# yamoling/lle

Hardware: AMD Instinct MI355X
Metric: env-steps/s (agents x envs x steps/s), level-6 batch 65536 (higher is better)
Workload: dtype u8

## Files before the change

### lle_amd/csrc/kernel_common.hpp

```cpp
#pragma once
#include <hip/hip_runtime.h>
#include <stdint.h>
#include <stdlib.h>

#include "kernels.h"
#include "obs_stream.hpp"
#include "step_logic.hpp"
#include "tables.h"

namespace lle {

enum Mode : int { MODE_STEP = 0, MODE_RESET = 1, MODE_SET_STATE = 2, MODE_OBSERVE = 3, MODE_SOURCES = 4, MODE_ENV_SOURCES = 5 };

__device__ __forceinline__ uint64_t wave_sum_u64(uint64_t v) {
#pragma unroll
    for (int o = 32; o >= 1; o >>= 1) {
        uint32_t lo = __shfl_xor((uint32_t)v, o, 64);
        uint32_t hi = __shfl_xor((uint32_t)(v >> 32), o, 64);
        v += ((uint64_t)hi << 32) | lo;
    }
    return v;
}

struct StepCounts { uint32_t steps, gems, exits, died, invalid, resets, bonus; };
__device__ __forceinline__ uint32_t wave_sum_u32(uint32_t v) {
#pragma unroll
    for (int o = 32; o >= 1; o >>= 1) v += __shfl_xor(v, o, 64);
    return v;
}
__device__ __forceinline__ int64_t stats_preload(const int64_t* __restrict__ stats, uint32_t wave_id, uint32_t lane) {
    return lane < 8 ? stats[(int64_t)wave_id * 8 + lane] : 0;
}
__device__ __forceinline__ void flush_stats(int64_t* __restrict__ stats, uint32_t wave_id, const StepCounts& c, int A, uint32_t lane,
                                            bool preloaded = false, int64_t old = 0) {
    const int64_t steps = wave_sum_u32(c.steps), gems = wave_sum_u32(c.gems), exits = wave_sum_u32(c.exits);
    const int64_t died = wave_sum_u32(c.died), invalid = wave_sum_u32(c.invalid), resets = wave_sum_u32(c.resets);
    const int64_t bonus = wave_sum_u32(c.bonus);
    const int64_t v = lane == 0 ? steps : lane == 1 ? steps * A : lane == 2 ? gems : lane == 3 ? exits : lane == 4 ? died
                    : lane == 5 ? invalid : lane == 6 ? resets : gems + exits - died + bonus;
    if (preloaded) {
        if (lane < 8) stats[(int64_t)wave_id * 8 + lane] = old + v;
    } else if (lane == 0) {
        int64_t* out = stats + (int64_t)wave_id * 8;
        out[0] += steps; out[1] += steps * A; out[2] += gems; out[3] += exits; out[4] += died;
        out[5] += invalid; out[6] += resets; out[7] += gems + exits - died + bonus;
    }
}

template <int AM>
__device__ __forceinline__ void store_u16_record(uint16_t* __restrict__ base, int64_t env, const uint32_t (&v)[AM]) {
    uint32_t* __restrict__ w = reinterpret_cast<uint32_t*>(base) + env * (AM / 2);
#pragma unroll
    for (int k = 0; k < AM / 2; k++) w[k] = (v[2 * k] & 0xFFFFu) | (v[2 * k + 1] << 16);
}
template <int AM>
__device__ __forceinline__ void load_u8_record(const uint8_t* __restrict__ base, int64_t env, uint32_t (&out)[AM]) {
    const uint32_t* __restrict__ w = reinterpret_cast<const uint32_t*>(base) + env * (AM / 4);
#pragma unroll
    for (int k = 0; k < AM / 4; k++) {
        const uint32_t v = w[k];
#pragma unroll
        for (int q = 0; q < 4; q++) out[4 * k + q] = (v >> (8 * q)) & 0xFFu;
    }
}
template <int AM>
__device__ __forceinline__ void store_u8_record(uint8_t* __restrict__ base, int64_t env, const uint32_t (&v)[AM]) {
    uint32_t* __restrict__ w = reinterpret_cast<uint32_t*>(base) + env * (AM / 4);
#pragma unroll
    for (int k = 0; k < AM / 4; k++)
        w[k] = (v[4 * k] & 0xFFu) | ((v[4 * k + 1] & 0xFFu) << 8) | ((v[4 * k + 2] & 0xFFu) << 16) | (v[4 * k + 3] << 24);
}

}
```

### lle_amd/csrc/step_kernel.hpp

```cpp
#pragma once
#include "kernel_common.hpp"
#include "partial_stream.hpp"
#include "step_lanes.hpp"

namespace lle {


__device__ __forceinline__ EnvOutputs load_uniform(const EnvOutputs* p) {
    static_assert(sizeof(EnvOutputs) == 64, "one s_load_dwordx16");
    typedef uint32_t u32x16 __attribute__((ext_vector_type(16)));
    u32x16 w;
    asm volatile("s_load_dwordx16 %0, %1, 0x0\n\ts_waitcnt lgkmcnt(0)" : "=s"(w) : "s"(p) : "memory");
    EnvOutputs o;
    __builtin_memcpy(&o, &w, sizeof o);
    return o;
}

constexpr size_t KERNARG_ENV_OUT = ((sizeof(BatchPtrs) + alignof(LaunchArgs) - 1) / alignof(LaunchArgs)) * alignof(LaunchArgs) + offsetof(LaunchArgs, out);
__device__ __forceinline__ const EnvOutputs* kernarg_env_out() {
    return reinterpret_cast<const EnvOutputs*>((const char*)__builtin_amdgcn_kernarg_segment_ptr() + KERNARG_ENV_OUT);
}

__device__ __forceinline__ uint32_t park_uniform(uint32_t s) {
    uint32_t v;
// ... 167 lines not shown
    const uint32_t head2_lo = (HEAD && PES) ? hdr->pes_head2_lo : 0u, head2_n = (HEAD && PES && head_n) ? head2_n_map : 0u;
    uint4 head_v = {0u, 0u, 0u, 0u};
    if (HEAD) {
        const uint32_t q_lay = hdr->off_cell_lay, q_lds = hdr->lds_table_bytes, q_ig = initp->gems;
        const uint64_t q_ib = initp->bits;
        asm("" : "+s"(head_lo) : "s"(h_HW), "s"(h_obs_stride), "s"(h_n_chunks), "s"(h_D), "s"(h_enabled), "s"(h_off_cell_meta), "s"(h_off_dyn), "s"(h_off_template),
                                 "s"(head_n_map), "s"(q_lay), "s"(q_lds), "s"(q_ig), "s"((uint32_t)q_ib), "s"((uint32_t)(q_ib >> 32)), "s"(A), "s"(W),
                                 "s"((uint32_t)hdr->obs_supported));
#pragma unroll
        for (int b = 0; b < LR; b++)
            if (!BM && b < L) asm("" : "+s"(head_lo) : "s"(h_beam_full[b]), "s"(h_init_beams[b]));
        if (BM) asm("" : "+s"(head_lo) : "s"(h_chain));
        if (PES) asm("" : "+s"(head_lo) : "s"(h_off_recolour), "s"(h_off_bare), "s"(h_off_elems), "s"(h_n_elems), "s"(head2_lo), "s"(head2_n_map), "s"((uint32_t)hdr->ext_bytes),
                                          "s"((uint32_t)hdr->recolour_exact));
        if (ENV_OUT) asm("" : "+s"(head_lo) : "s"(h_G), "s"(h_H));
        if (lane < head_n + head2_n)
            head_v = reinterpret_cast<const uint4*>(tables + (PES ? h_off_bare : h_off_template))[lane < head_n ? head_lo + lane : head2_lo + (lane - head_n)];
        LLE_LOAD_STATE();
    }
    uint32_t bt_full = 0u, bt_init = 0u;
    if (BM && (int)threadIdx.x < L) {
        bt_full = hdr->beam_full[threadIdx.x];
        bt_init = initp->beams[threadIdx.x];
    }
    const uint32_t tab_off = hdr->off_cell_lay;
    const uint32_t tab_cells = ((hdr->off_dyn - tab_off) + 1023u) & ~1023u;
    const uint32_t tab_bytes = PARTIAL ? (tab_cells < hdr->lds_table_bytes ? tab_cells : hdr->lds_table_bytes)
                                       : (split ? hdr->lds_split_table_bytes : hdr->lds_table_bytes);
    const bool use_sets = PARTIAL && K.win_sets != nullptr;
    const uint32_t ext_bytes = PES ? hdr->ext_bytes : (use_sets ? win_sets_bytes(hdr->HW) : 0u);
    constexpr int PB = CAN_SPLIT ? 8 : 1;
    const uint32_t cpw = (h_n_chunks + waves_per_wg - 1u) / waves_per_wg;
    const uint32_t c_lo = wave_in_wg * cpw < h_n_chunks ? wave_in_wg * cpw : h_n_chunks;
    const uint32_t c_hi = c_lo + cpw < h_n_chunks ? c_lo + cpw : h_n_chunks;
    uint32_t pre_bits[PB];
    uint32_t pre_neg = 0xFFFFFFFFu;
#pragma unroll
    for (int q = 0; q < PB; q++) pre_bits[q] = 0u;
    if (CAN_SPLIT && split) {
        const uint16_t* __restrict__ bits = reinterpret_cast<const uint16_t*>(tables + sizeof(MapHeader)) + c_lo;
#pragma unroll
        for (int q = 0; q < PB; q++)
            if (lane + 64u * q < c_hi - c_lo) pre_bits[q] = bits[lane + 64u * q];
        if (lane < TMPL_NEG_MAX) pre_neg = reinterpret_cast<const uint32_t*>(tables + sizeof(MapHeader) + tmpl_bits_bytes(h_n_chunks))[lane];
        if (!HEAD) LLE_LOAD_STATE();
    }
    if (PES) copy_tables2_to_lds<HEAD>(tables + tab_off, tab_bytes, tables + h_off_bare, ext_bytes, lds, lane, wave_in_wg, waves_per_wg);
    else if (use_sets) copy_tables2_to_lds(tables + tab_off, tab_bytes, K.win_sets + (uint64_t)map_idx * win_table_bytes(hdr->HW), ext_bytes, lds, lane, wave_in_wg, waves_per_wg);
    else if (CAN_SPLIT && GEN && split && (K.flags & LAUNCH_PACKED_TABLES))
        expand_packed_tables(tables + hdr->off_packed, lds, h_HW, hdr->packed_n_lay, h_off_cell_meta - tab_off, h_off_dyn - tab_off, h_off_template - h_off_dyn,
                             threadIdx.x, blockDim.x);
    else copy_tables_to_lds<HEAD>(tables + tab_off, lds, tab_bytes, lane, wave_in_wg, waves_per_wg);
    constexpr uint32_t bt_bytes = BM ? 2u * LM * 4u : 0u;
    uint32_t* beam_tab = reinterpret_cast<uint32_t*>(lds + tab_bytes + ext_bytes);
    if (BM && (int)threadIdx.x < L) {
        beam_tab[threadIdx.x] = bt_full;
        beam_tab[LM + threadIdx.x] = bt_init;
    }
    const uint32_t pm_bytes = PARTIAL ? (use_sets ? 0u : partial_bitmap_bytes(hdr->H, (uint32_t)W)) + 32u : 0u;
    uint32_t* const part_bm = reinterpret_cast<uint32_t*>(lds + tab_bytes + ext_bytes + bt_bytes);
    uint8_t* const part_col = lds + tab_bytes + ext_bytes + bt_bytes + (pm_bytes - 32u);
    if (PARTIAL) {
        for (uint32_t w = threadIdx.x; w < (pm_bytes - 32u) / 4u; w += blockDim.x) part_bm[w] = 0u;
        if ((int)threadIdx.x < L) part_col[threadIdx.x] = hdr->beam_colour[threadIdx.x];
    }
    LLE_STAMP(7);
    if (HEAD) {
        __builtin_amdgcn_s_waitcnt(0x0F70);
        const uint32_t hgroup = MODE != 6 ? 1u : ((K.flags & LAUNCH_HEAD_GROUP4) ? 4u : ((K.flags & LAUNCH_HEAD_GROUP2) ? 2u : 1u));
        const uint32_t wt = K.flags & LAUNCH_WRITE_THROUGH;
        if (__builtin_expect(hot, 1)) {
            if (head_n && n_rows) store_heads_hot(P.obs, h_obs_stride, env0, n_rows, head_lo, head_n, head_v, lane, head2_lo, head2_n);
            asm volatile("s_waitcnt lgkmcnt(0)\n\ts_barrier" ::: "memory");
        } else if (hgroup == 1u) {
            if (head_n && n_rows) store_heads_cold(P.obs, h_obs_stride, env0, n_rows, head_lo, head_n, head_v, lane, LLE_ROT(), head2_lo, head2_n, wt);
            asm volatile("s_waitcnt lgkmcnt(0)\n\ts_barrier" ::: "memory");
        } else {
            asm volatile("s_waitcnt lgkmcnt(0)\n\ts_barrier" ::: "memory");
            if (head_n && (wave_in_wg & (hgroup - 1u)) == 0u) {
                for (uint32_t q = 0; q < hgroup && wave_in_wg + q < waves_per_wg; q++) {
                    const int64_t e0q = env0 + (int64_t)q * EPW;
                    int64_t nq = K.env_limit - e0q;
                    nq = nq < 0 ? 0 : (nq > (int64_t)EPW ? (int64_t)EPW : nq);
                    if (nq > 0) store_heads_cold(P.obs, h_obs_stride, e0q, (uint32_t)nq, head_lo, head_n, head_v, lane, 0u, 0u, 0u, wt);
                }
            }
        }
    } else {
        __syncthreads();
        if (!(CAN_SPLIT && split)) LLE_LOAD_STATE();
    }

    const uint32_t pk_wave = HEAD ? park_uniform(wave_id) : 0u, pk_env_lo = HEAD ? park_uniform((uint32_t)env0) : 0u,
                   pk_env_hi = HEAD ? park_uniform((uint32_t)((uint64_t)env0 >> 32)) : 0u;
    const uint64_t* cell_lay = reinterpret_cast<const uint64_t*>(lds);
    const uint32_t* cell_meta = reinterpret_cast<const uint32_t*>(lds + (h_off_cell_meta - tab_off));
    const uint64_t* dyn = reinterpret_cast<const uint64_t*>(lds + (h_off_dyn - tab_off));
    const uint16_t* dyn_chunks = PES ? reinterpret_cast<const uint16_t*>(lds + tab_bytes + (h_off_dyn_chunks - h_off_bare))
                                     : reinterpret_cast<const uint16_t*>(lds + (h_off_dyn_chunks - tab_off));
    const uint32_t scr_stride = (uint32_t)(L + A + 2 + (PES ? CW : 0)) | 1u;
    const uint32_t part_pitch = PARTIAL ? (((uint32_t)(A * (2 * A + 3)) * K.partial_k * K.partial_k + 15u) & ~15u) : 0u;
    const uint32_t row_area = PARTIAL ? K.partial_E * part_pitch + 16u : h_obs_stride;
    const uint32_t priv_bytes = row_area + (PARTIAL ? ((EPW * scr_stride * 4u + 15u) & ~15u) : 64u * scr_stride * 4u) + (PES ? PES_WAVE_EXTRA_BYTES : 0u);
    int8_t* tmpl = reinterpret_cast<int8_t*>(lds + tab_bytes + ext_bytes + bt_bytes + pm_bytes + wave_in_wg * priv_bytes);
    uint32_t* scratch = reinterpret_cast<uint32_t*>(tmpl + row_area);
    const int8_t* bare = reinterpret_cast<const int8_t*>(lds + tab_bytes);
    const uint32_t* elems = reinterpret_cast<const uint32_t*>(lds + tab_bytes + (h_off_elems - h_off_bare));
    if (split) {
        tmpl = reinterpret_cast<int8_t*>(lds + tab_bytes + bt_bytes + wave_in_wg * cpw * 16u);
        scratch = reinterpret_cast<uint32_t*>(lds + tab_bytes + bt_bytes + waves_per_wg * cpw * 16u) + wave_in_wg * EPW * scr_stride;
        uint4* mine = reinterpret_cast<uint4*>(tmpl);
        if (hdr->off_tmpl_bits) {
            auto expand = [](uint32_t b) {
                return uint4{((b & 15u) * 0x00204081u) & 0x01010101u, (((b >> 4) & 15u) * 0x00204081u) & 0x01010101u,
                             (((b >> 8) & 15u) * 0x00204081u) & 0x01010101u, ((b >> 12) * 0x00204081u) & 0x01010101u};
            };
#pragma unroll
            for (int q = 0; q < PB; q++)
                if (lane + 64u * q < c_hi - c_lo) mine[lane + 64u * q] = expand(pre_bits[q]);
            const uint16_t* __restrict__ bits = reinterpret_cast<const uint16_t*>(tables + sizeof(MapHeader)) + c_lo;
            for (uint32_t c = lane + 64u * PB; c < c_hi - c_lo; c += 64) mine[c] = expand(bits[c]);
            if (lane < hdr->tmpl_neg_n && pre_neg >= c_lo * 16u && pre_neg < c_hi * 16u) tmpl[pre_neg - c_lo * 16u] = (int8_t)-1;
        } else {
            const uint4* __restrict__ pristine = reinterpret_cast<const uint4*>(tables + h_off_template) + c_lo;
            for (uint32_t c = lane; c < c_hi - c_lo; c += 64) mine[c] = pristine[c];
        }
    } else if (PARTIAL) {
        if (!use_sets) partial_bitmap_fill(part_bm, cell_lay, cell_meta, (int)hdr->H, W);
    } else {
        const uint4* pristine = PES ? reinterpret_cast<const uint4*>(bare) : reinterpret_cast<const uint4*>(lds + (h_off_template - tab_off));
        uint4* mine = reinterpret_cast<uint4*>(tmpl);
        for (uint32_t c = lane; c < h_n_chunks; c += 64) mine[c] = pristine[c];
    }
    uint32_t* const bm = scratch + grp * scr_stride + 1;
    if (HEAD && BM) {
        if (env_ok) {
#pragma unroll
            for (int k = 0; k < BPL; k++)
                if ((int)a + k * G < L) bm[(int)a + k * G] = bm_pre[k];
        }
    } else if (BM && env_ok) {
        for (int b = (int)a; b < L; b += G) bm[b] = p_beams[b];
    }
    wave_sync();
    if (!HEAD) __builtin_amdgcn_s_waitcnt(0x0F70);
    LLE_STAMP(1);

    uint32_t alive = (uint32_t)raw_bits & 0xFFFFu, arrived = (uint32_t)(raw_bits >> 16) & 0xFFFFu, occ = (uint32_t)(raw_bits >> 32) & 0xFFFFu;
    uint32_t ghost = (uint32_t)(raw_bits >> GHOST_SHIFT);
    const uint32_t enabled = PES ? env_enabled : h_enabled, max_layers = h_max_layers;
    LLE_STAMP(2);

    StepCounts cnt = {0, 0, 0, 0, 0, 0, 0};
    constexpr bool CNT_LDS = ROLL && PES && G >= 2;
    uint32_t* const cnt_lds = scratch + 64u * scr_stride + grp * 8u;
    if (CNT_LDS && env_ok && a == 0) {
#pragma unroll
        for (int q = 0; q < 7; q++) cnt_lds[q] = 0u;
    }
    const uint32_t n_steps = ROLL ? (K.n_steps ? K.n_steps : 1u) : 1u;
    for (uint32_t it = 0; it < n_steps; it++) {
    const uint64_t t_now = K.t + it;
    uint8_t* __restrict__ actions_out = P.actions;
    uint32_t* __restrict__ reward_out = P.reward;
    int8_t* __restrict__ obs_out = P.obs;
    if (ROLL && K.ring_slots) {
        uint32_t slot = (uint32_t)K.ring_pos + it;
        while (slot >= K.ring_slots) slot -= K.ring_slots;
        actions_out = K.ring_actions + (int64_t)slot * K.ring_env_count * As;
        reward_out = K.ring_reward + (int64_t)slot * K.ring_env_count;
        obs_out = K.ring_obs + (int64_t)slot * K.ring_env_count * (int64_t)LLE_PITCH();
    }

    uint32_t was_reset = 0;
    if (K.flags & STEP_AUTO_RESET) {
        const bool over = env_ok && ((alive | ghost) != amask || arrived == amask);
        pos = (over && me) ? init_pos_a : pos;
        avail = (over && me) ? init_avail_a : avail;
        alive = over ? ((uint32_t)init_bits & 0xFFFFu) : alive;
        arrived = over ? ((uint32_t)(init_bits >> 16) & 0xFFFFu) : arrived;
        occ = over ? ((uint32_t)(init_bits >> 32) & 0xFFFFu) : occ;
        ghost = over ? 0u : ghost;
        gems = over ? init_gems : gems;
#pragma unroll
        for (int b = 0; b < LR; b++)
            if (!BM && b < L && !(PES && shared_init))
                beams[b] = over ? (PES ? (PRE_BEAMS ? env_init_beams[b] : P.init_beams[env_ok ? env * L + b : 0]) : h_init_beams[b]) : beams[b];
        if (BM && over && !(PES && shared_init))
            for (int b = (int)a; b < L; b += G) bm[b] = PES ? P.init_beams[env * L + b] : beam_tab[LM + b];
        if (PES && shared_init && __ballot(over) != 0ull) {
            const uint32_t* rtab0 = reinterpret_cast<const uint32_t*>(lds + tab_bytes + (h_off_recolour - h_off_bare));
            if (!BM) {
#pragma unroll
                for (int b = 0; b < LR; b++)
                    if (b < L) {
                        const uint32_t c = (colw[b >> 2] >> ((b & 3) * 8)) & 0xFFu;
                        const uint32_t m = ((env_enabled >> b) & 1u) ? rtab0[b * (A + 1) + 1 + (int)(c < (uint32_t)A ? c : 0u)] : 0u;
                        beams[b] = over ? m : beams[b];
                    }
            } else if (over) {
                for (int b = (int)a; b < L; b += G) {
                    const uint32_t c = (colw[b >> 2] >> ((b & 3) * 8)) & 0xFFu;
                    bm[b] = ((env_enabled >> b) & 1u) ? rtab0[b * (A + 1) + 1 + (int)(c < (uint32_t)A ? c : 0u)] : 0u;
                }
            }
        }
        was_reset = over ? 1u : 0u;
        if (PES && !ROLL && (K.flags & STEP_RECOLOUR_RESETS) && __ballot(over) != 0ull) {
            const uint32_t* rtab = reinterpret_cast<const uint32_t*>(lds + tab_bytes + (h_off_recolour - h_off_bare));
            const uint64_t rkey = action_step_key(K.seed ^ RECOLOUR_SALT, t_now);
#pragma unroll
            for (int b = 0; b < LM; b++) {
                if (b < L) {
                    const uint32_t* row = rtab + b * (A + 1);
                    const uint32_t ok = row[0] & amask;
                    const uint32_t field = action_field(action_hash_pair(rkey, (uint64_t)(K.env_offset + env), (uint32_t)b >> 1), (uint32_t)b);
                    const uint32_t k = (field * (uint32_t)__popc(ok)) >> 16;
                    const bool mine = ((ok >> a) & 1u) != 0u && (uint32_t)__popc(ok & ((1u << a) - 1u)) == k;
                    const uint32_t pick = grp_or<G>(mine ? a + 1u : 0u);
                    const uint32_t sh = (uint32_t)(b & 3) * 8u, old_c = (colw[b >> 2] >> sh) & 0xFFu;
                    const uint32_t c = (over && pick) ? pick - 1u : old_c;
                    colw[b >> 2] = (colw[b >> 2] & ~(0xFFu << sh)) | (c << sh);
                    if (over && a == 0) P.init_beams[env * L + b] = ((env_enabled >> b) & 1u) ? row[1u + (c < (uint32_t)A ? c : 0u)] : 0u;
                }
            }
            if (over && a == 0) {
#pragma unroll
                for (int q = 0; q < CWM; q++)
                    if (q < CW) reinterpret_cast<uint32_t*>(P.src_colour)[env * CW + q] = colw[q];
            }
        }
    }

    uint32_t act = 4u;
    if (K.flags & STEP_SAMPLE_ACTIONS) {
        const uint32_t hp = action_hash_pair(action_step_key(K.seed, t_now), (uint64_t)(K.env_offset + env), a >> 1);
        act = sample_action(avail, action_field(hp, a));
        if (me) small_store(&actions_out[env * As + a], (uint8_t)act);
    } else if (!ROLL) {
        act = act_given;
        if (me && K.actions_in) P.actions[env * As + a] = (uint8_t)act;
    } else if (K.actions_in) {
        if (me) {
            act = (uint32_t)K.actions_in[env * A + a];
            P.actions[env * As + a] = (uint8_t)act;
        }
    } else if (me) {
        act = (uint32_t)actions_out[env * As + a];
    }

    uint64_t evw[NW];
    uint32_t n_ev, meta_step, err;
    bool stepped;
    step_lanes<G, LR, ML1, PES, CWM, true, BM>(cell_lay, cell_meta, A, L, W, max_layers, h_beam_full, a, me, env_ok, enabled, colw, act, pos, avail,
                                               alive, arrived, occ, gems, beams, err, evw, n_ev, meta_step, stepped, nullptr, bm, beam_tab, h_chain);
    LLE_STAMP(3);

    const uint32_t wave_id_l = HEAD ? unpark_uniform(pk_wave) : wave_id;
    const int64_t env0_l = HEAD ? (int64_t)(((uint64_t)unpark_uniform(pk_env_hi) << 32) | unpark_uniform(pk_env_lo)) : env0;
#define LLE_ROT_L() ((ROLL && PES) ? 0u : row_rotation(wave_id_l, EPW, n_here, K.flags))
    auto post_step = [&]() {
    LLE_ENV_LATE(env_p);
    if (stepped) avail_lanes<G>(a, me, pos, occ, alive, arrived, meta_step, avail);
#pragma unroll
    for (int k = 0; k < NW; k++) evw[k] = grp_or64<G>(evw[k]);
    if (env_ok && a == 0) {
        small_store(LLE_LATE(err, env_p), (uint8_t)err);
        small_store(LLE_LATE(evcount, env_p), (uint8_t)(n_ev | (was_reset << 7)));
        {
            uint8_t* row = LLE_LATE(events, env_p * 2 * As);
            if (G >= 2) {
                uint32_t* __restrict__ w = reinterpret_cast<uint32_t*>(row);
#pragma unroll
                for (int k = 0; k < G / 2; k++) small_store(&w[k], (uint32_t)(evw[k >> 1] >> ((k & 1) * 32)));
            } else {
                small_store(reinterpret_cast<uint16_t*>(row), (uint16_t)evw[0]);
            }
        }
        small_store(LLE_LATE(done, env_p), (uint8_t)(((alive | ghost) != amask || arrived == amask) ? 1 : 0));
        uint32_t n_died = 0, n_gem = 0;
#pragma unroll
        for (int k = 0; k < NW; k++) {
            n_died += (uint32_t)__popcll(evw[k] & 0x2020202020202020ull);
            n_gem += (uint32_t)__popcll(evw[k] & 0x1010101010101010ull);
        }
        const uint32_t n_exit = n_ev - n_died - n_gem;
        const uint32_t bonus = (err == 0 && arrived == amask) ? 1u : 0u;
        small_store(&reward_out[env], n_gem | (n_exit << 8) | (n_died << 16) | (bonus << 24));
        if (CNT_LDS) {
            const uint32_t add[7] = {1u, n_gem, n_exit, n_died, err != 0 ? 1u : 0u, was_reset, bonus};
#pragma unroll
            for (int q = 0; q < 7; q++) __hip_atomic_fetch_add(&cnt_lds[q], add[q], __ATOMIC_RELAXED, __HIP_MEMORY_SCOPE_WAVEFRONT);
        } else {
            cnt.steps += 1u; cnt.gems += n_gem; cnt.exits += n_exit; cnt.died += n_died;
            cnt.invalid += err != 0 ? 1u : 0u; cnt.resets += was_reset; cnt.bonus += bonus;
        }
    }
    if (ENV_OUT && K.env_out) {
        const EnvOutputs O = EARLY_OUT ? O_early : load_uniform(kernarg_env_out());
        const int n_gems = (int)h_G, len = 3 * A + n_gems;
        if (me) {
            const int64_t ia = env * A + a;
            if (O.alive) small_store(&O.alive[ia], (uint8_t)((alive >> a) & 1u));
            if (O.arrived) small_store(&O.arrived[ia], (uint8_t)((arrived >> a) & 1u));
            if (O.available) {
                uint8_t* o = O.available + ia * 5;
#pragma unroll
                for (int k = 0; k < 5; k++) small_store(&o[k], (uint8_t)((avail >> k) & 1u));
            }
        }
#define LLE_STATE_IJ()                                               \
    float fi = (float)(pos & 0xFFu), fj = (float)(pos >> 8);         \
    if (O.normalize_state) {                                         \
        fi = (float)((double)(pos & 0xFFu) / (double)h_H);           \
        fj = (float)((double)(pos >> 8) / (double)W);                \
    }
        if (HEAD) {
            const uint32_t st_off = (EPW * scr_stride * 4u + 15u) & ~15u;
            const bool staged = !split && O.state && (len & 3) == 0 && (reinterpret_cast<uintptr_t>(O.state) & 15u) == 0u &&
                                st_off + EPW * (uint32_t)len * 4u <= 64u * scr_stride * 4u;
            if (O.state) {
                float* st = staged ? reinterpret_cast<float*>(reinterpret_cast<uint8_t*>(scratch) + st_off) + grp * (uint32_t)len : O.state + env * len;
                if (me) {
                    LLE_STATE_IJ()
                    st[2 * a] = fi;
                    st[2 * a + 1] = fj;
                    st[2 * A + n_gems + (int)a] = ((alive >> a) & 1u) ? 1.0f : 0.0f;
                }
                if (env_ok)
                    for (int g = (int)a; g < n_gems; g += G) st[2 * A + g] = ((gems >> g) & 1u) ? 1.0f : 0.0f;
                if (staged) {
                    wave_sync();
                    const float4* src4 = reinterpret_cast<const float4*>(reinterpret_cast<uint8_t*>(scratch) + st_off);
                    float4* dst4 = reinterpret_cast<float4*>(O.state + env0_l * len);
                    const uint32_t n4 = n_here > 0 ? (uint32_t)n_here * (uint32_t)len / 4u : 0u;
                    for (uint32_t c = lane; c < n4; c += 64u) dst4[c] = src4[c];
                    wave_sync();
                }
            }
        } else {
            if (me && O.state) {
                float* st = O.state + env * len;
                LLE_STATE_IJ()
                small_store(&st[2 * a], fi);
                small_store(&st[2 * a + 1], fj);
                small_store(&st[2 * A + n_gems + (int)a], ((alive >> a) & 1u) ? 1.0f : 0.0f);
            }
            if (env_ok && O.state)
                for (int g = (int)a; g < n_gems; g += G) small_store(&O.state[env * len + 2 * A + g], ((gems >> g) & 1u) ? 1.0f : 0.0f);
        }
#undef LLE_STATE_IJ
        if (env_ok && a == 0) {
            if (O.done) small_store(&O.done[env], (uint8_t)(((alive | ghost) != amask || arrived == amask) ? 1 : 0));
            if (O.reward) {
                uint32_t n_died = 0, n_gem = 0;
#pragma unroll
                for (int k = 0; k < NW; k++) {
                    n_died += (uint32_t)__popcll(evw[k] & 0x2020202020202020ull);
                    n_gem += (uint32_t)__popcll(evw[k] & 0x1010101010101010ull);
                }
                const float gem = (float)n_gem, died = (float)n_died, ex = (float)(n_ev - n_died - n_gem);
                const float bonus = (err == 0 && arrived == amask) ? 1.0f : 0.0f;
                if (O.reward_kind == 0) {
                    small_store(&O.reward[env], gem + ex - died + bonus);
                } else {
                    const bool dead = n_died > 0;
                    float* o = O.reward + env * 4;
                    small_store(&o[0], dead ? 0.f : gem); small_store(&o[1], dead ? 0.f : ex); small_store(&o[2], -died); small_store(&o[3], dead ? 0.f : bonus);
                }
            }
        }
    }
    };

    if (env_ok && a == 0) {
        uint32_t* sc = scratch + grp * scr_stride;
        sc[0] = 0u;
#pragma unroll
        for (int b = 0; b < LR; b++)
            if (!BM && b < L) sc[1 + b] = beams[b];
        sc[L + 1] = ~gems;
        if (PES) {
#pragma unroll
            for (int q = 0; q < CWM; q++)
                if (q < CW) sc[L + 2 + A + q] = colw[q];
        }
    }
    if (me) scratch[grp * scr_stride + L + 2 + a] = PARTIAL ? pos : a * h_HW + cell_of(pos, W);
    if (split) {
        asm volatile("s_waitcnt lgkmcnt(0)\n\ts_barrier" ::: "memory");
    } else {
        wave_sync();
    }
    LLE_STAMP(4);
    const bool post_first = ROLL || PARTIAL || (K.flags & LAUNCH_POST_FIRST) || (!(K.flags & LAUNCH_POST_LAST) && blockIdx.x * 4u >= gridDim.x * 3u);
    if (post_first) post_step();

    const uint32_t et = LLE_ET();
    if (split) {
        if (write_obs) {
            const int64_t wg_env0 = K.env_base + (int64_t)(blk * waves_per_wg) * EPW;
            int64_t n_wg = K.env_limit - wg_env0;
            n_wg = n_wg < 0 ? 0 : (n_wg > (int64_t)(waves_per_wg * EPW) ? (int64_t)(waves_per_wg * EPW) : n_wg);
            const uint32_t* records = reinterpret_cast<const uint32_t*>(lds + tab_bytes + bt_bytes + waves_per_wg * cpw * 16u);
            dispatch_stream<!HEAD>(K.flags, [&](auto wt_, auto wide_) {
                constexpr bool WT = decltype(wt_)::value, WIDE = decltype(wide_)::value;
                if (CAN_INCR && incr) write_observations_split<WT, true, WIDE>(A, L, h_D, c_lo, c_hi, LLE_PITCH(), dyn, tmpl, records, scr_stride, obs_out, wg_env0, n_wg, lane, dyn_chunks, h_n_dyn_chunks, et);
                else write_observations_split<WT, false, WIDE>(A, L, h_D, c_lo, c_hi, LLE_PITCH(), dyn, tmpl, records, scr_stride, obs_out, wg_env0, n_wg, lane, nullptr, 0u, et);
            });
        }
        if (ROLL && n_steps > 1) asm volatile("s_waitcnt lgkmcnt(0)\n\ts_barrier" ::: "memory");
    } else if (PARTIAL) {
        asm volatile("s_waitcnt lgkmcnt(0)\n\ts_barrier" ::: "memory");
        const EnvOutputs O = load_uniform(kernarg_env_out());
        if (O.partial && n_here > 0)
            write_partial<true>(A, L, W, (int)K.partial_k, part_pitch, K.partial_E, h_max_layers, cell_lay, cell_meta, part_bm, part_col, tmpl, scratch,
                                scr_stride, O.partial, env0_l, n_here, lane, use_sets ? reinterpret_cast<const uint64_t*>(lds + tab_bytes) : nullptr, et);
    } else if (HEAD && write_obs && n_here > 0) {
        uint32_t lflags = K.flags;
        asm volatile("" : "+s"(lflags));
        if (__builtin_expect((lflags & HOT_RULES) == LAUNCH_WRITE_THROUGH, 1)) {
            if (PES)
                write_observations_env<true, true, false, false, HP_HOT>(A, L, h_HW, h_n_elems, h_n_chunks, LLE_PITCH(), elems, bare, tmpl, scratch, scr_stride, obs_out, env0_l, n_here,
                                                                         lane, nullptr, 0xFFFFFFFFu, head_lo, head_n, 0u, nullptr, 0u, head2_lo, head2_n, et);
            else
                write_observations<true, true, false, false, HP_HOT>(A, L, h_D, h_n_chunks, LLE_PITCH(), dyn, tmpl, scratch, scr_stride, obs_out, env0_l, n_here, lane, head_lo, head_n,
                                                                     0u, nullptr, 0u, et);
        } else {
            if (PES)
                write_observations_env<false, true, false, false, HP_COLD>(A, L, h_HW, h_n_elems, h_n_chunks, LLE_PITCH(), elems, bare, tmpl, scratch, scr_stride, obs_out, env0_l, n_here,
                                                                           lane, nullptr, 0xFFFFFFFFu, head_lo, head_n, LLE_ROT_L(), nullptr, 0u, head2_lo, head2_n, et,
                                                                           K.flags & LAUNCH_WRITE_THROUGH);
            else
                write_observations<false, true, false, false, HP_COLD>(A, L, h_D, h_n_chunks, LLE_PITCH(), dyn, tmpl, scratch, scr_stride, obs_out, env0_l, n_here, lane, head_lo, head_n,
                                                                       LLE_ROT_L(), nullptr, 0u, et, K.flags & LAUNCH_WRITE_THROUGH);
        }
    } else if (!HEAD && write_obs && n_here > 0) {
        dispatch_stream<!HEAD>(K.flags, [&](auto wt_, auto wide_) {
            constexpr bool WT = decltype(wt_)::value, WIDE = decltype(wide_)::value;
            if (PES && CAN_INCR && incr)
                write_observations_env<WT, false, true, WIDE>(A, L, h_HW, h_n_elems, h_n_chunks, LLE_PITCH(), elems, bare, tmpl, scratch, scr_stride, obs_out, env0_l, n_here,
                                                              lane, nullptr, 0xFFFFFFFFu, 0u, 0u, LLE_ROT_L(), dyn_chunks, h_n_dyn_chunks, 0u, 0u, et);
            else if (PES)
                write_observations_env<WT, HEAD, false, WIDE>(A, L, h_HW, h_n_elems, h_n_chunks, LLE_PITCH(), elems, bare, tmpl, scratch, scr_stride, obs_out, env0_l, n_here,
                                                              lane, nullptr, 0xFFFFFFFFu, head_lo, head_n, LLE_ROT_L(), nullptr, 0u, head2_lo, head2_n, et);
            else if (CAN_INCR && incr)
                write_observations<WT, false, true, WIDE>(A, L, h_D, h_n_chunks, LLE_PITCH(), dyn, tmpl, scratch, scr_stride, obs_out, env0_l, n_here, lane, 0u, 0u, LLE_ROT_L(),
                                                          dyn_chunks, h_n_dyn_chunks, et);
            else
                write_observations<WT, HEAD, false, WIDE>(A, L, h_D, h_n_chunks, LLE_PITCH(), dyn, tmpl, scratch, scr_stride, obs_out, env0_l, n_here, lane, head_lo, head_n,
                                                          LLE_ROT_L(), nullptr, 0u, et);
        });
    }
    wave_sync();
    if (!post_first) post_step();
    }
    LLE_STAMP(5);

    LLE_ENV_LATE(env_f);
    if (me) {
        small_store(LLE_LATE(pos, env_f * As + a), (uint16_t)pos);
        small_store(LLE_LATE(avail, env_f * As + a), (uint8_t)avail);
    }
    if (env_ok && a == 0) {
        small_store(LLE_LATE(bits, env_f), (uint64_t)alive | ((uint64_t)arrived << 16) | ((uint64_t)occ << 32) | ((uint64_t)ghost << GHOST_SHIFT));
        small_store(LLE_LATE(gems, env_f), gems);
        uint32_t* const beams_out = LLE_LATE(beams, env_f * L);
#pragma unroll
        for (int b = 0; b < LR; b++)
            if (!BM && b < L) small_store(&beams_out[b], beams[b]);
    }
    if (BM && env_ok) {
        uint32_t* const beams_out = LLE_LATE(beams, env_f * L);
        for (int b = (int)a; b < L; b += G) small_store(&beams_out[b], bm[b]);
#undef LLE_LATE
#undef LLE_ENV_LATE
#undef LLE_LOAD_STATE
#undef LLE_ROT
#undef LLE_ROT_L
#undef LLE_ET
#undef LLE_PITCH
    }
    if (CNT_LDS && env_ok && a == 0) {
        cnt.steps = cnt_lds[0]; cnt.gems = cnt_lds[1]; cnt.exits = cnt_lds[2]; cnt.died = cnt_lds[3];
        cnt.invalid = cnt_lds[4]; cnt.resets = cnt_lds[5]; cnt.bonus = cnt_lds[6];
    }
    flush_stats(P.stats, HEAD ? unpark_uniform(pk_wave) : wave_id, cnt, A, lane, PRE_STATS, stats_old);
    if (STAMPED && stamps) {
        asm volatile("s_waitcnt vmcnt(0)" ::: "memory");
        LLE_STAMP(6);
    }
}

template <int G, int LM, int MODE, bool ML1, int LX = -1>
static hipError_t launch_step_glp(const BatchPtrs& P, const LaunchArgs& K, uint32_t n_waves, uint32_t wpw, uint32_t lds, hipStream_t stream) {
    static std::atomic<uint32_t> noted{0};
    const uint32_t note_bit = (K.flags & LAUNCH_DRY_RUN) ? 2u : 1u;
    if (!(noted.load(std::memory_order_relaxed) & note_bit)) {
        noted.fetch_or(note_bit, std::memory_order_relaxed);
        debug_note(debug_key(DBG_STEP, G, LM, MODE, ML1, LX), (K.flags & LAUNCH_DRY_RUN) != 0);
    }
    if (K.flags & LAUNCH_DRY_RUN) return hipSuccess;
    dim3 grid((n_waves + wpw - 1) / wpw), block(64 * wpw);
    if (lds > 64 * 1024) {
        static LdsGrant granted;
        hipError_t e = granted.ensure(reinterpret_cast<const void*>(&step_kernel<G, LM, MODE, ML1, LX>), lds);
        if (e != hipSuccess) return e;
    }
    hipLaunchKernelGGL((step_kernel<G, LM, MODE, ML1, LX>), grid, block, lds, stream, P, K);
    return hipGetLastError();
}
template <int MODE, int G, int LM>
static hipError_t launch_step_mode_gl(const BatchPtrs& P, const LaunchArgs& K, uint32_t n_waves, uint32_t wpw, uint32_t lds, hipStream_t stream) {
    const bool ml1 = (K.flags & LAUNCH_SINGLE_LAYER) != 0;
    if constexpr (LM == 4) {
        if (ml1) {
#define LLE_STEP_LX(X) case X: return launch_step_glp<G, 4, MODE, true, X>(P, K, n_waves, wpw, lds, stream);
            switch (K.n_sources) { LLE_STEP_LX(0) LLE_STEP_LX(1) LLE_STEP_LX(2) LLE_STEP_LX(3) LLE_STEP_LX(4) default: return hipErrorInvalidValue; }
#undef LLE_STEP_LX
        }
        return launch_step_glp<G, 4, MODE, false>(P, K, n_waves, wpw, lds, stream);
    } else {
        return ml1 ? launch_step_glp<G, LM, MODE, true>(P, K, n_waves, wpw, lds, stream)
                   : launch_step_glp<G, LM, MODE, false>(P, K, n_waves, wpw, lds, stream);
    }
}
template <int MODE, int G>
static hipError_t launch_step_mode_g(int lm, const BatchPtrs& P, const LaunchArgs& K, uint32_t n_waves, uint32_t wpw, uint32_t lds, hipStream_t stream) {
    if constexpr (MODE == 6 || MODE == 7 || MODE == 8 || MODE == 9) {
        if (lm == 4) return launch_step_mode_gl<MODE, G, 4>(P, K, n_waves, wpw, lds, stream);
        if (lm == 8) return launch_step_mode_gl<MODE, G, 8>(P, K, n_waves, wpw, lds, stream);
        return hipErrorInvalidValue;
    } else {
        switch (lm) {
            case 4: return launch_step_mode_gl<MODE, G, 4>(P, K, n_waves, wpw, lds, stream);
            case 8: return launch_step_mode_gl<MODE, G, 8>(P, K, n_waves, wpw, lds, stream);
            case 16: return launch_step_mode_gl<MODE, G, 16>(P, K, n_waves, wpw, lds, stream);
            default: return launch_step_mode_gl<MODE, G, 32>(P, K, n_waves, wpw, lds, stream);
        }
    }
}
template <int MODE>
static hipError_t launch_step_mode(int G, int lm, const BatchPtrs& P, const LaunchArgs& K, uint32_t n_waves, uint32_t wpw, uint32_t lds, hipStream_t stream) {
    switch (G) {
        case 1: return launch_step_mode_g<MODE, 1>(lm, P, K, n_waves, wpw, lds, stream);
        case 2: return launch_step_mode_g<MODE, 2>(lm, P, K, n_waves, wpw, lds, stream);
        case 4: return launch_step_mode_g<MODE, 4>(lm, P, K, n_waves, wpw, lds, stream);
        case 8: return launch_step_mode_g<MODE, 8>(lm, P, K, n_waves, wpw, lds, stream);
        default: return launch_step_mode_g<MODE, 16>(lm, P, K, n_waves, wpw, lds, stream);
    }
}

}
```

### lle_amd/csrc/step_logic.hpp

```cpp
#pragma once
#include <stdint.h>

#include "tables.h"

#if defined(__HIPCC__)
#define LLE_HD __host__ __device__ __forceinline__
#else
#define LLE_HD inline
#endif

namespace lle {

LLE_HD uint64_t mix64(uint64_t x) {
    x ^= x >> 30; x *= 0xBF58476D1CE4E5B9ULL;
    x ^= x >> 27; x *= 0x94D049BB133111EBULL;
    x ^= x >> 31;
    return x;
}
LLE_HD uint32_t rotl32(uint32_t x, uint32_t s) { return (x << (s & 31u)) | (x >> ((32u - s) & 31u)); }
LLE_HD uint64_t action_step_key(uint64_t seed, uint64_t t) { return mix64(seed + 0x9E3779B97F4A7C15ULL * (t + 1)); }
LLE_HD uint32_t action_hash_pair(uint64_t key, uint64_t env, uint32_t pair) {
    uint32_t h = ((uint32_t)key ^ ((uint32_t)env * 0x9E3779B1u)) + rotl32((uint32_t)(key >> 32) ^ (uint32_t)(env >> 32), 15u) +
                 rotl32(0xC2B2AE35u, 3u * pair + 1u);
    h ^= h >> 16; h *= 0x7FEB352Du;
    h ^= h >> 15; h *= 0x846CA68Bu;
    h ^= h >> 16;
    return h;
}
LLE_HD uint32_t action_field(uint32_t pair_hash, uint32_t agent) { return (pair_hash >> (16u * (agent & 1u))) & 0xFFFFu; }

LLE_HD uint32_t popc5(uint32_t m) {
#if defined(__HIP_DEVICE_COMPILE__)
    return (uint32_t)__popc(m);
#else
    return (uint32_t)__builtin_popcount(m);
#endif
}
LLE_HD uint32_t sample_action(uint32_t mask, uint32_t field16) {
    mask &= 31u;
    const uint32_t k = (field16 * popc5(mask)) >> 16;
    uint32_t act = 4;
#pragma unroll
    for (int b = 4; b >= 0; b--) {
        const uint32_t below = popc5(mask & ((1u << b) - 1u));
        act = (((mask >> b) & 1u) && below == k) ? (uint32_t)b : act;
    }
    return act;
}

struct MapView {
    const uint64_t* cell_lay;
    const uint32_t* cell_meta;
    const MapHeader* hdr;
    int W, A, L, G;
    uint32_t enabled;
    uint32_t max_layers;
    bool per_env;
    uint32_t colw[MAX_SOURCES / 4];
    uint32_t chain = 0;
};

template <int NWORDS>
LLE_HD uint32_t colour_get(const uint32_t (&colw)[NWORDS], uint32_t b) {
    uint32_t w = 0;
#pragma unroll
    for (int k = 0; k < NWORDS; k++) w = ((b >> 2) == (uint32_t)k) ? colw[k] : w;
    return (w >> ((b & 3u) * 8u)) & 0xFFu;
}
template <int NWORDS, int NL = MAX_CELL_LAYERS>
LLE_HD uint64_t recolour_lay(uint64_t lay, const uint32_t (&colw)[NWORDS]) {
    uint64_t out = NL < MAX_CELL_LAYERS ? (lay & ~((1ull << (16 * NL)) - 1ull)) : 0ull;
#pragma unroll
    for (int q = 0; q < NL; q++) {
        uint32_t e = lay_entry(lay, (int)q);
        const uint32_t c = colour_get<NWORDS>(colw, lay_word(e));
        e = (e & LAY_VALID) ? ((e & 0x7FFu) | (c << 11)) : e;
        out |= (uint64_t)e << (16 * q);
    }
    return out;
}

template <int AM, int LM>
struct Env {
    uint32_t pos[AM];
    uint32_t alive, arrived, occ;
    uint32_t gems;
    uint32_t beams[LM];
};

template <int AM>
struct Events {
    static constexpr int NW = (2 * AM + 7) / 8;
    uint64_t w[NW];
    uint32_t n;
    LLE_HD void clear() {
#pragma unroll
        for (int k = 0; k < NW; k++) w[k] = 0;
        n = 0;
    }
    LLE_HD void push_if(bool c, uint32_t type, uint32_t agent) {
        const uint64_t byte = c ? (uint64_t)((type << 4) | agent) : 0ull;
        const uint32_t word = n >> 3, sh = (n & 7u) * 8u;
#pragma unroll
        for (int k = 0; k < NW; k++) w[k] |= (NW == 1 || word == (uint32_t)k) ? (byte << sh) : 0ull;
        n += c ? 1u : 0u;
    }
};

LLE_HD uint32_t cell_of(uint32_t p, int W) { return (p & 0xFFu) * (uint32_t)W + (p >> 8); }

template <int AM>
struct Cells {
    uint64_t lay[AM];
    uint32_t meta[AM];
};
template <int AM>
LLE_HD void load_cells(const MapView& mv, const uint32_t (&pos)[AM], Cells<AM>& out) {
#pragma unroll
    for (int a = 0; a < AM; a++) {
        const uint32_t c = (a < mv.A) ? cell_of(pos[a], mv.W) : 0u;
        out.lay[a] = mv.cell_lay[c];
        if (mv.per_env) out.lay[a] = recolour_lay<MAX_SOURCES / 4>(out.lay[a], mv.colw);
        out.meta[a] = mv.cell_meta[c];
    }
}

template <int LM>
LLE_HD uint32_t beam_get(const uint32_t (&b)[LM], uint32_t idx) {
    uint32_t r = 0;
#pragma unroll
    for (int k = 0; k < LM; k++) r = (idx == (uint32_t)k) ? b[k] : r;
    return r;
}
template <int LM>
LLE_HD void beam_set_if(uint32_t (&b)[LM], uint32_t idx, bool c, uint32_t v) {
#pragma unroll
    for (int k = 0; k < LM; k++) b[k] = (c && idx == (uint32_t)k) ? v : b[k];
}

template <int LM>
LLE_HD void chain_rest(uint32_t (&beams)[LM], uint32_t b, bool c, bool fill, uint32_t chain) {
    if (!chain) return;
    bool carry = false;
#pragma unroll
    for (int k = 0; k < LM; k++) {
        carry = carry && ((chain >> k) & 1u);
        beams[k] = carry ? (fill ? 0xFFFFFFFFu : 0u) : beams[k];
        carry = carry || (c && b == (uint32_t)k);
    }
}

template <int LM>
LLE_HD void lasers_leave(uint32_t (&beams)[LM], uint64_t lay, bool doit, const MapView& mv) {
    for (uint32_t k = 0; k < mv.max_layers; k++) {
        const uint32_t e = lay_entry(lay, (int)k);
        const uint32_t b = lay_word(e), off = lay_bit(e);
        const uint32_t m = beam_get<LM>(beams, b);
        const bool c = doit && (e & LAY_VALID) && !((m >> off) & 1u) && ((mv.enabled >> b) & 1u);
        beam_set_if<LM>(beams, b, c, m | (0xFFFFFFFFu << off));
        chain_rest<LM>(beams, b, c, true, mv.chain);
    }
}

template <int LM>
LLE_HD void lasers_pre_enter(uint32_t (&beams)[LM], uint64_t lay, uint32_t agent, bool alive, const MapView& mv) {
    for (uint32_t k = 0; k < mv.max_layers; k++) {
        const uint32_t e = lay_entry(lay, (int)k);
        const uint32_t b = lay_word(e), off = lay_bit(e), colour = lay_colour(e);
        const bool c = alive && (e & LAY_VALID) && colour == agent && ((mv.enabled >> b) & 1u);
        const uint32_t m = beam_get<LM>(beams, b);
        beam_set_if<LM>(beams, b, c, m & ((1u << off) - 1u));
        chain_rest<LM>(beams, b, c, false, mv.chain);
    }
}

template <int LM>
LLE_HD bool lasers_block(const uint32_t (&beams)[LM], uint64_t lay, uint32_t agent, const MapView& mv) {
    bool blocked = false;
    for (uint32_t k = 0; k < mv.max_layers; k++) {
        const uint32_t e = lay_entry(lay, (int)k);
        const uint32_t b = lay_word(e), off = lay_bit(e), colour = lay_colour(e);
        const uint32_t m = beam_get<LM>(beams, b);
// ... 196 lines not shown
```

Before: 13.58 billion.

## Pack step counters into two words and reduce with DPP row ops

Replaces the shuffle-based wave reductions with DPP row operations plus four readlanes. In the non-rollout path it packs the seven per-step counters into two 32-bit words, so only two wave sums are needed instead of seven. It also moves the final state stores and the stats flush into the per-step body so they can issue earlier. The packed form depends on every 8-bit field staying in range, which a static_assert checks for a single step per wave.

After: 14.15 billion (median of 6 runs). +4.2%, better.

```diff
diff --git a/lle_amd/csrc/kernel_common.hpp b/lle_amd/csrc/kernel_common.hpp
--- a/lle_amd/csrc/kernel_common.hpp
+++ b/lle_amd/csrc/kernel_common.hpp
@@ -12,30 +12,40 @@
 
 enum Mode : int { MODE_STEP = 0, MODE_RESET = 1, MODE_SET_STATE = 2, MODE_OBSERVE = 3, MODE_SOURCES = 4, MODE_ENV_SOURCES = 5 };
 
+template <int CTRL>
+__device__ __forceinline__ uint32_t dpp_row_u32(uint32_t v) {
+    return (uint32_t)__builtin_amdgcn_update_dpp(0, (int)v, CTRL, 0xF, 0xF, true);
+}
+constexpr int DPP_QUAD_XOR1 = 0xB1, DPP_QUAD_XOR2 = 0x4E, DPP_ROW_HALF_MIRROR = 0x141, DPP_ROW_MIRROR = 0x140;
+__device__ __forceinline__ uint32_t wave_sum_u32(uint32_t v) {
+    v += dpp_row_u32<DPP_QUAD_XOR1>(v);
+    v += dpp_row_u32<DPP_QUAD_XOR2>(v);
+    v += dpp_row_u32<DPP_ROW_HALF_MIRROR>(v);
+    v += dpp_row_u32<DPP_ROW_MIRROR>(v);
+    return (uint32_t)__builtin_amdgcn_readlane((int)v, 0) + (uint32_t)__builtin_amdgcn_readlane((int)v, 16) +
+           (uint32_t)__builtin_amdgcn_readlane((int)v, 32) + (uint32_t)__builtin_amdgcn_readlane((int)v, 48);
+}
+template <int CTRL>
+__device__ __forceinline__ uint64_t dpp_row_u64(uint64_t v) {
+    return ((uint64_t)dpp_row_u32<CTRL>((uint32_t)(v >> 32)) << 32) | dpp_row_u32<CTRL>((uint32_t)v);
+}
 __device__ __forceinline__ uint64_t wave_sum_u64(uint64_t v) {
+    v += dpp_row_u64<DPP_QUAD_XOR1>(v);
+    v += dpp_row_u64<DPP_QUAD_XOR2>(v);
+    v += dpp_row_u64<DPP_ROW_HALF_MIRROR>(v);
+    v += dpp_row_u64<DPP_ROW_MIRROR>(v);
+    uint64_t s = 0;
 #pragma unroll
-    for (int o = 32; o >= 1; o >>= 1) {
-        uint32_t lo = __shfl_xor((uint32_t)v, o, 64);
-        uint32_t hi = __shfl_xor((uint32_t)(v >> 32), o, 64);
-        v += ((uint64_t)hi << 32) | lo;
-    }
-    return v;
+    for (int r = 0; r < 64; r += 16)
+        s += ((uint64_t)(uint32_t)__builtin_amdgcn_readlane((int)(uint32_t)(v >> 32), r) << 32) | (uint32_t)__builtin_amdgcn_readlane((int)(uint32_t)v, r);
+    return s;
 }
 
-struct StepCounts { uint32_t steps, gems, exits, died, invalid, resets, bonus; };
-__device__ __forceinline__ uint32_t wave_sum_u32(uint32_t v) {
-#pragma unroll
-    for (int o = 32; o >= 1; o >>= 1) v += __shfl_xor(v, o, 64);
-    return v;
-}
 __device__ __forceinline__ int64_t stats_preload(const int64_t* __restrict__ stats, uint32_t wave_id, uint32_t lane) {
     return lane < 8 ? stats[(int64_t)wave_id * 8 + lane] : 0;
 }
-__device__ __forceinline__ void flush_stats(int64_t* __restrict__ stats, uint32_t wave_id, const StepCounts& c, int A, uint32_t lane,
-                                            bool preloaded = false, int64_t old = 0) {
-    const int64_t steps = wave_sum_u32(c.steps), gems = wave_sum_u32(c.gems), exits = wave_sum_u32(c.exits);
-    const int64_t died = wave_sum_u32(c.died), invalid = wave_sum_u32(c.invalid), resets = wave_sum_u32(c.resets);
-    const int64_t bonus = wave_sum_u32(c.bonus);
+__device__ __forceinline__ void store_stats(int64_t* __restrict__ stats, uint32_t wave_id, const StepCounts& c, int A, uint32_t lane, bool preloaded, int64_t old) {
+    const int64_t steps = c.steps, gems = c.gems, exits = c.exits, died = c.died, invalid = c.invalid, resets = c.resets, bonus = c.bonus;
     const int64_t v = lane == 0 ? steps : lane == 1 ? steps * A : lane == 2 ? gems : lane == 3 ? exits : lane == 4 ? died
                     : lane == 5 ? invalid : lane == 6 ? resets : gems + exits - died + bonus;
     if (preloaded) {
@@ -45,6 +55,16 @@
         out[0] += steps; out[1] += steps * A; out[2] += gems; out[3] += exits; out[4] += died;
         out[5] += invalid; out[6] += resets; out[7] += gems + exits - died + bonus;
     }
+}
+__device__ __forceinline__ void flush_stats(int64_t* __restrict__ stats, uint32_t wave_id, const StepCounts& c, int A, uint32_t lane,
+                                            bool preloaded = false, int64_t old = 0) {
+    const StepCounts sums = {wave_sum_u32(c.steps), wave_sum_u32(c.gems), wave_sum_u32(c.exits), wave_sum_u32(c.died),
+                             wave_sum_u32(c.invalid), wave_sum_u32(c.resets), wave_sum_u32(c.bonus)};
+    store_stats(stats, wave_id, sums, A, lane, preloaded, old);
+}
+__device__ __forceinline__ void flush_stats_packed(int64_t* __restrict__ stats, uint32_t wave_id, uint32_t reward_word, uint32_t flags_word, int A, uint32_t lane,
+                                                   bool preloaded, int64_t old) {
+    store_stats(stats, wave_id, stat_unpack(wave_sum_u32(reward_word), wave_sum_u32(flags_word)), A, lane, preloaded, old);
 }
 
 template <int AM>
diff --git a/lle_amd/csrc/step_kernel.hpp b/lle_amd/csrc/step_kernel.hpp
--- a/lle_amd/csrc/step_kernel.hpp
+++ b/lle_amd/csrc/step_kernel.hpp
@@ -343,12 +343,33 @@
     LLE_STAMP(2);
 
     StepCounts cnt = {0, 0, 0, 0, 0, 0, 0};
+    static_assert(stat_fields_fit(64u / G, G) && stat_fields_fit(64u / G, 2u * G), "the packed counters of a wavefront's single step must fit 8-bit fields");
+    uint32_t cnt_reward = 0u, cnt_flags = 0u;
+    constexpr bool TAIL_IN_POST = !ROLL && !(MODE == 7 && BM);
     constexpr bool CNT_LDS = ROLL && PES && G >= 2;
     uint32_t* const cnt_lds = scratch + 64u * scr_stride + grp * 8u;
     if (CNT_LDS && env_ok && a == 0) {
 #pragma unroll
         for (int q = 0; q < 7; q++) cnt_lds[q] = 0u;
     }
+    auto final_state = [&](int64_t env_f) {
+        if (me) {
+            small_store(LLE_LATE(pos, env_f * As + a), (uint16_t)pos);
+            small_store(LLE_LATE(avail, env_f * As + a), (uint8_t)avail);
+        }
+        if (env_ok && a == 0) {
+            small_store(LLE_LATE(bits, env_f), (uint64_t)alive | ((uint64_t)arrived << 16) | ((uint64_t)occ << 32) | ((uint64_t)ghost << GHOST_SHIFT));
+            small_store(LLE_LATE(gems, env_f), gems);
+            uint32_t* const beams_out = LLE_LATE(beams, env_f * L);
+#pragma unroll
+            for (int b = 0; b < LR; b++)
+                if (!BM && b < L) small_store(&beams_out[b], beams[b]);
+        }
+        if (BM && env_ok) {
+            uint32_t* const beams_out = LLE_LATE(beams, env_f * L);
+            for (int b = (int)a; b < L; b += G) small_store(&beams_out[b], bm[b]);
+        }
+    };
     const uint32_t n_steps = ROLL ? (K.n_steps ? K.n_steps : 1u) : 1u;
     for (uint32_t it = 0; it < n_steps; it++) {
     const uint64_t t_now = K.t + it;
@@ -477,11 +498,15 @@
         }
         const uint32_t n_exit = n_ev - n_died - n_gem;
         const uint32_t bonus = (err == 0 && arrived == amask) ? 1u : 0u;
-        small_store(&reward_out[env], n_gem | (n_exit << 8) | (n_died << 16) | (bonus << 24));
+        const uint32_t reward_word = stat_pack_reward(n_gem, n_exit, n_died, bonus);
+        small_store(&reward_out[env], reward_word);
         if (CNT_LDS) {
             const uint32_t add[7] = {1u, n_gem, n_exit, n_died, err != 0 ? 1u : 0u, was_reset, bonus};
 #pragma unroll
             for (int q = 0; q < 7; q++) __hip_atomic_fetch_add(&cnt_lds[q], add[q], __ATOMIC_RELAXED, __HIP_MEMORY_SCOPE_WAVEFRONT);
+        } else if (!ROLL) {
+            cnt_reward = reward_word;
+            cnt_flags = stat_pack_flags(1u, err != 0 ? 1u : 0u, was_reset);
         } else {
             cnt.steps += 1u; cnt.gems += n_gem; cnt.exits += n_exit; cnt.died += n_died;
             cnt.invalid += err != 0 ? 1u : 0u; cnt.resets += was_reset; cnt.bonus += bonus;
@@ -561,6 +586,10 @@
                 }
             }
         }
+    }
+    if (TAIL_IN_POST) {
+        final_state(env_p);
+        if (PRE_STATS) flush_stats_packed(P.stats, wave_id_l, cnt_reward, cnt_flags, A, lane, true, stats_old);
     }
     };
 
@@ -648,22 +677,10 @@
     }
     LLE_STAMP(5);
 
-    LLE_ENV_LATE(env_f);
-    if (me) {
-        small_store(LLE_LATE(pos, env_f * As + a), (uint16_t)pos);
-        small_store(LLE_LATE(avail, env_f * As + a), (uint8_t)avail);
-    }
-    if (env_ok && a == 0) {
-        small_store(LLE_LATE(bits, env_f), (uint64_t)alive | ((uint64_t)arrived << 16) | ((uint64_t)occ << 32) | ((uint64_t)ghost << GHOST_SHIFT));
-        small_store(LLE_LATE(gems, env_f), gems);
-        uint32_t* const beams_out = LLE_LATE(beams, env_f * L);
-#pragma unroll
-        for (int b = 0; b < LR; b++)
-            if (!BM && b < L) small_store(&beams_out[b], beams[b]);
-    }
-    if (BM && env_ok) {
-        uint32_t* const beams_out = LLE_LATE(beams, env_f * L);
-        for (int b = (int)a; b < L; b += G) small_store(&beams_out[b], bm[b]);
+    if (!TAIL_IN_POST) {
+        LLE_ENV_LATE(env_f);
+        final_state(env_f);
+    }
 #undef LLE_LATE
 #undef LLE_ENV_LATE
 #undef LLE_LOAD_STATE
@@ -671,12 +688,12 @@
 #undef LLE_ROT_L
 #undef LLE_ET
 #undef LLE_PITCH
-    }
     if (CNT_LDS && env_ok && a == 0) {
         cnt.steps = cnt_lds[0]; cnt.gems = cnt_lds[1]; cnt.exits = cnt_lds[2]; cnt.died = cnt_lds[3];
         cnt.invalid = cnt_lds[4]; cnt.resets = cnt_lds[5]; cnt.bonus = cnt_lds[6];
     }
-    flush_stats(P.stats, HEAD ? unpark_uniform(pk_wave) : wave_id, cnt, A, lane, PRE_STATS, stats_old);
+    if (ROLL) flush_stats(P.stats, wave_id, cnt, A, lane);
+    else if (!PRE_STATS || !TAIL_IN_POST) flush_stats_packed(P.stats, HEAD ? unpark_uniform(pk_wave) : wave_id, cnt_reward, cnt_flags, A, lane, PRE_STATS, stats_old);
     if (STAMPED && stamps) {
         asm volatile("s_waitcnt vmcnt(0)" ::: "memory");
         LLE_STAMP(6);
diff --git a/lle_amd/csrc/step_logic.hpp b/lle_amd/csrc/step_logic.hpp
--- a/lle_amd/csrc/step_logic.hpp
+++ b/lle_amd/csrc/step_logic.hpp
@@ -28,6 +28,16 @@
     return h;
 }
 LLE_HD uint32_t action_field(uint32_t pair_hash, uint32_t agent) { return (pair_hash >> (16u * (agent & 1u))) & 0xFFFFu; }
+
+struct StepCounts { uint32_t steps, gems, exits, died, invalid, resets, bonus; };
+constexpr uint32_t STAT_FIELD_MAX = 255u;
+LLE_HD uint32_t stat_pack_reward(uint32_t n_gem, uint32_t n_exit, uint32_t n_died, uint32_t bonus) { return n_gem | (n_exit << 8) | (n_died << 16) | (bonus << 24); }
+LLE_HD uint32_t stat_pack_flags(uint32_t steps, uint32_t invalid, uint32_t resets) { return steps | (invalid << 8) | (resets << 16); }
+LLE_HD StepCounts stat_unpack(uint32_t reward_sum, uint32_t flags_sum) {
+    return StepCounts{flags_sum & 0xFFu, reward_sum & 0xFFu, (reward_sum >> 8) & 0xFFu, (reward_sum >> 16) & 0xFFu,
+                      (flags_sum >> 8) & 0xFFu, (flags_sum >> 16) & 0xFFu, reward_sum >> 24};
+}
+constexpr bool stat_fields_fit(uint32_t n_envs, uint32_t per_env_max) { return n_envs * per_env_max <= STAT_FIELD_MAX; }
 
 LLE_HD uint32_t popc5(uint32_t m) {
 #if defined(__HIP_DEVICE_COMPILE__)
```
